# guo-research-group/Blurry-Edges

Hardware: AMD Instinct MI355X
Metric: patch-pairs/s (local CNN + render + depth) on 21x21 synth (higher is better)
Workload: dtype f32; 1 GPU; configs[1]: batch of 4096 synthetic 21x21 two-aperture patch pairs per GPU (8192 CNN patches): LocalStage inference + pass-A colour solve + depth solve; pairs_per_gpu=4096, streams=2, weights=portable-generator random init (no checkpoint offline)

## Files before the change

blurry-edges_amd/csrc/be_conv_pm_bf6.hip:

```cpp
#include "be_common.h"
#include "be_device_math.h"
#include "be_split_bf16.h"
#include <cstdlib>

namespace {

using be::bf6::bf16x8;
using be::bf6::f32x4;
using be::bf6::split8;
using be::bf6::PS_BLOCK;
using be::bf6::ps_slot;
typedef float f32x16 __attribute__((ext_vector_type(16)));
typedef __attribute__((address_space(3))) void* lds_ptr_t;
typedef const __attribute__((address_space(1))) void* glb_ptr_t;

constexpr int L0_BM = 128, L0_BKT = 16, L0_STAGES = 4;
constexpr int L0_ABYTES = L0_BM * L0_BKT * 4, L0_BBYTES = PS_BLOCK * 2, L0_STAGE = L0_ABYTES + L0_BBYTES;

struct PmBf6Args {
    const float* x;
    const float* x2;
    const float* planes;
    const float* bias;
    float* y;
    int Nimg, H, W, HW, Cin, Cin2, Cout, ldy, act, groups, ncc;
    int64_t istride, istride2;
};

__global__ __launch_bounds__(256, 2)
void k_conv_pm_bf6(PmBf6Args a) {
    constexpr int BM = L0_BM, BKT = L0_BKT, NS = L0_STAGES, ABYTES = L0_ABYTES, BBYTES = L0_BBYTES, STAGE = L0_STAGE;
    extern __shared__ __attribute__((aligned(16))) float smem_l0[];
    char* const lds = reinterpret_cast<char*>(smem_l0);

    const int bid = blockIdx.x;
    const int xcd = bid & 7, t = bid >> 3;
    const int grp = (t / a.HW) * 8 + xcd;
    if (grp >= a.groups) return;
    const int img0 = grp * BM;
    int py, px;
    {
        const int idx = t % a.HW, ni = (a.H - 2) * (a.W - 2);
        if (idx < ni) { py = 1 + idx / (a.W - 2); px = 1 + idx % (a.W - 2); }
        else {
            const int e = idx - ni;
            if (e < a.W) { py = 0; px = e; }
            else if (e < 2 * a.W) { py = a.H - 1; px = e - a.W; }
            else if (e < 2 * a.W + a.H - 2) { px = 0; py = 1 + e - 2 * a.W; }
            else { px = a.W - 1; py = 1 + e - 2 * a.W - (a.H - 2); }
        }
    }
    unsigned long long tap_list = 0;
    int ntap = 0;
#pragma unroll
    for (int k = 0; k < 9; ++k) {
        const bool ok = (unsigned)(py + k / 3 - 1) < (unsigned)a.H && (unsigned)(px + k % 3 - 1) < (unsigned)a.W;
        if (ok) { tap_list |= (unsigned long long)k << (4 * ntap); ++ntap; }
    }

    const int tid = threadIdx.x;
    const int wave = __builtin_amdgcn_readfirstlane(tid >> 6), lane = tid & 63;
    const int li = lane & 31, lh = lane >> 5;
    float bias_v[3];
#pragma unroll
    for (int j = 0; j < 3; ++j) {
        const int c = j * 32 + li;
        bias_v[j] = (c < a.Cout && a.bias) ? a.bias[c] : 0.0f;
    }
    const int srow = lane >> 2, sq = (lane & 3) ^ ((lane >> 4) & 3);
    unsigned a_off[2], a_off2[2];
#pragma unroll
    for (int p = 0; p < 2; ++p) {
        const int r = (2 * wave + p) * 16 + srow;
        const int rr = img0 + r < a.Nimg ? r : 0;
        a_off[p] = (unsigned)(rr * a.istride + 4 * sq) * 4u;
        a_off2[p] = (unsigned)(rr * a.istride2 + 4 * sq) * 4u;
    }
    const float* xpix = a.x + (int64_t)img0 * a.istride + (py * a.W + px) * a.Cin;
    const float* x2pix = a.x2 ? a.x2 + (int64_t)img0 * a.istride2 + (py * a.W + px) * a.Cin2 : nullptr;
    const char* wt = reinterpret_cast<const char*>(a.planes) + lane * 16;

    const int n_main = a.ncc * ntap * 2;
    const int total = n_main + (a.x2 ? a.Cin2 / BKT : 0);
    int w_cc = 0, w_j = 0, w_sub = 0, w_k = 0, l_buf = 0;
#define L0_DMA()                                                                                                \
    do {                                                                                                        \
        char* st_ = lds + l_buf * STAGE;                                                                        \
        const char* xs_;                                                                                        \
        int chunk_;                                                                                             \
        unsigned o0_, o1_;                                                                                      \
        if (w_k < n_main) {                                                                                     \
            const int tap_ = (int)((tap_list >> (4 * w_j)) & 15ull);                                            \
            const int ty_ = (tap_ * 11) >> 5, tx_ = tap_ - 3 * ty_;                         \
            xs_ = reinterpret_cast<const char*>(xpix + ((ty_ - 1) * a.W + tx_ - 1) * a.Cin + w_cc * 32 + w_sub * BKT); \
            chunk_ = (w_cc * 9 + tap_) * 2 + w_sub;                                                             \
            o0_ = a_off[0]; o1_ = a_off[1];                                                                     \
        } else {                                                                                                \
            const int k2_ = w_k - n_main;                                                                       \
            xs_ = reinterpret_cast<const char*>(x2pix + k2_ * BKT);                                             \
            chunk_ = a.ncc * 18 + k2_;                                                                          \
            o0_ = a_off2[0]; o1_ = a_off2[1];                                                                   \
        }                                                                                                       \
        __builtin_amdgcn_global_load_lds((glb_ptr_t)(xs_ + o0_), (lds_ptr_t)(st_ + (2 * wave) * 1024), 16, 0, 0);     \
        __builtin_amdgcn_global_load_lds((glb_ptr_t)(xs_ + o1_), (lds_ptr_t)(st_ + (2 * wave + 1) * 1024), 16, 0, 0); \
        const char* ws_ = wt + (int64_t)chunk_ * BBYTES;                                                        \
        _Pragma("unroll") for (int p_ = 0; p_ < 3; ++p_)                                                        \
            __builtin_amdgcn_global_load_lds((glb_ptr_t)(ws_ + (3 * wave + p_) * 1024),                         \
                                             (lds_ptr_t)(st_ + ABYTES + (3 * wave + p_) * 1024), 16, 0, 0);     \
        if (w_k + 1 < total) {                                           \
            ++w_k;                                                                                              \
            if (++w_sub == 2) { w_sub = 0; if (++w_j == ntap) { w_j = 0; ++w_cc; } }                            \
        }                                                                                                       \
        l_buf = (l_buf + 1) % NS;                                                                               \
    } while (0)

    const int fsw = (li >> 2) & 3;
    const int a_fr0 = ((wave * 32 + li) * BKT + 4 * ((2 * lh) ^ fsw)) * 4;
    const int a_fr1 = ((wave * 32 + li) * BKT + 4 * ((2 * lh + 1) ^ fsw)) * 4;
    const int b_fr = ABYTES + li * 32 + ps_slot(li, lh) * 16;
    f32x16 acc[3];
#pragma unroll
    for (int j = 0; j < 3; ++j)
#pragma unroll
        for (int r = 0; r < 16; ++r) acc[j][r] = 0.0f;
    bf16x8 ap[3], bp[3][3];
    int r_buf = 0;
#define L0_FRAGS()                                                                                              \
    do {                                                                                                        \
        const char* sb_ = lds + r_buf * STAGE;                                                                  \
        const f32x4 af0_ = *reinterpret_cast<const f32x4*>(sb_ + a_fr0);                                        \
        const f32x4 af1_ = *reinterpret_cast<const f32x4*>(sb_ + a_fr1);                                        \
        _Pragma("unroll") for (int p_ = 0; p_ < 3; ++p_)                                                        \
            _Pragma("unroll") for (int j_ = 0; j_ < 3; ++j_)                                                    \
                bp[p_][j_] = *reinterpret_cast<const bf16x8*>(sb_ + b_fr + p_ * 4096 + j_ * 32 * 32);           \
        split8(af0_, af1_, ap[0], ap[1], ap[2]);                                                                \
        r_buf = (r_buf + 1) % NS;                                                                               \
    } while (0)

    __builtin_amdgcn_sched_barrier(0);
    L0_DMA();
    L0_DMA();
    L0_DMA();
    __builtin_amdgcn_s_waitcnt(0x0F75);
    __builtin_amdgcn_s_barrier();
    L0_FRAGS();
    bool landed = true;
    for (int kc = 0; kc < total; ++kc) {
        if (!landed) __builtin_amdgcn_s_waitcnt(0x0F75);
        landed = false;
        __builtin_amdgcn_s_barrier();
        L0_DMA();
        __builtin_amdgcn_sched_barrier(0);
        {
            constexpr int PA[6] = {2, 0, 1, 1, 0, 0}, PB[6] = {0, 2, 1, 0, 1, 0};
#pragma unroll
            for (int p = 0; p < 6; ++p)
#pragma unroll
                for (int j = 0; j < 3; ++j)
                    acc[j] = __builtin_amdgcn_mfma_f32_32x32x16_bf16(ap[PA[p]], bp[PB[p]][j], acc[j], 0, 0, 0);
            L0_FRAGS();
        }
        __builtin_amdgcn_sched_barrier(0);
    }
#undef L0_DMA
#undef L0_FRAGS
    __builtin_amdgcn_s_waitcnt(0x0F70);
    __builtin_amdgcn_sched_barrier(0);

    const int64_t rs = (int64_t)a.HW * a.ldy;
    char* yt = reinterpret_cast<char*>(a.y + ((int64_t)img0 * a.HW + py * a.W + px) * a.ldy);
    const unsigned y_off = (unsigned)((wave * 32 + 4 * lh) * rs + li) * 4u;
    const bool interior = img0 + BM <= a.Nimg && a.Cout == 96;
#define L0_STORE(J)                                                                                             \
    do {                                                                                                        \
        float v_ = acc[J][r] + bias_v[J];                                                                       \
        if (a.act == 1) v_ = be::smish(v_); else if (a.act == 2) v_ = fmaxf(v_, 0.0f);                          \
        reinterpret_cast<float*>(yt + (size_t)ro * rs * 4 + y_off)[(J) * 32] = v_;                              \
    } while (0)
    if (interior) {
#pragma unroll
        for (int r = 0; r < 16; ++r) {
            const int ro = (r & 3) + 8 * (r >> 2);
#pragma unroll
            for (int j = 0; j < 3; ++j) L0_STORE(j);
        }
    } else {
#pragma unroll
        for (int j = 0; j < 3; ++j) {
            const bool c_ok = j * 32 + li < a.Cout;
#pragma unroll
            for (int r = 0; r < 16; ++r) {
                const int ro = (r & 3) + 8 * (r >> 2);
                if (c_ok && img0 + wave * 32 + 4 * lh + ro < a.Nimg) L0_STORE(j);
            }
        }
    }
#undef L0_STORE
}

inline int ktot_of(int cin, int cin2) { return 9 * cin + cin2; }
inline bool shape_ok(int cout, int cin, int cin2) {
    return cout > 0 && (cout + 31) / 32 * 32 == 96 && cin > 0 && cin % 32 == 0 && cin2 >= 0 && cin2 % 16 == 0;
}

}

bool be::l0_bf6_enabled() {
    static const bool f32 = (getenv("BE_L0_F32") != nullptr && atoi(getenv("BE_L0_F32")) != 0) ||
                            (getenv("BE_WINO_F32") != nullptr && atoi(getenv("BE_WINO_F32")) != 0);
    return !f32;
}

extern "C" size_t be_conv3x3_pm_bf6_packed_floats(int cout, int cin, int cin2) {
    if (!shape_ok(cout, cin, cin2)) return 0;
    return be_gemm_rows_bf6_packed_floats(cout, ktot_of(cin, cin2));
}

extern "C" int be_conv3x3_pm_bf6_pack_f32(const float* packed_w, int cout, int cin, int cin2, float* planes, void* stream) {
    BE_REQUIRE(packed_w && planes, "be_conv3x3_pm_bf6_pack_f32: null pointer");
    BE_REQUIRE(shape_ok(cout, cin, cin2),
               "be_conv3x3_pm_bf6_pack_f32: unsupported shape (cout %d: cout_pad32 must be 96; cin %d %% 32; cin2 %d %% 16)", cout, cin, cin2);
    return be_gemm_rows_bf6_pack_f32(packed_w, cout, ktot_of(cin, cin2), planes, stream);
}

int be::conv3x3_pm_bf6(const be_conv_desc* d, const float* x, const float* x2, int cin2, const float* planes, const float* bias,
                       float* y, int ldy, void* stream) {
    BE_REQUIRE(d && x && planes && y, "be_conv3x3_pm_bf6_f32: null pointer");
    BE_REQUIRE(d->ksize == 3 && d->n >= 0 && (unsigned)d->act <= 2u, "be_conv3x3_pm_bf6_f32: bad descriptor (ksize %d, n %d, act %d)",
               d->ksize, d->n, d->act);
    BE_REQUIRE(x2 || cin2 == 0, "be_conv3x3_pm_bf6_f32: cin2 %d without x2", cin2);
    BE_REQUIRE(shape_ok(d->cout, d->cin, cin2) && (!x2 || cin2 > 0),
               "be_conv3x3_pm_bf6_f32: unsupported shape (cout %d: cout_pad32 must be 96; cin %d %% 32; cin2 %d %% 16)", d->cout, d->cin, cin2);
    BE_REQUIRE(d->h >= 3 && d->w >= 3 && ldy >= d->cout, "be_conv3x3_pm_bf6_f32: unsupported map (h %d, w %d >= 3; ldy %d >= cout)",
               d->h, d->w, ldy);
    BE_REQUIRE(be::aligned16(x) && be::aligned16(x2) && be::aligned16(planes) && (reinterpret_cast<uintptr_t>(y) & 3u) == 0 &&
               (!bias || (reinterpret_cast<uintptr_t>(bias) & 3u) == 0),
               "be_conv3x3_pm_bf6_f32: x / x2 / planes must be 16-byte aligned, y / bias 4-byte");
    if (d->n == 0) return BE_OK;
    PmBf6Args a;
    a.x = x; a.x2 = x2; a.planes = planes; a.bias = bias; a.y = y;
    a.Nimg = d->n; a.H = d->h; a.W = d->w; a.HW = d->h * d->w; a.Cin = d->cin; a.Cin2 = x2 ? cin2 : 0; a.Cout = d->cout; a.ldy = ldy;
    a.act = d->act; a.ncc = d->cin / 32;
    a.istride = (int64_t)a.HW * d->cin;
    a.istride2 = (int64_t)a.HW * a.Cin2;
    const int64_t span = 256 * 4 * (a.istride > a.istride2 ? a.istride : a.istride2);
    BE_REQUIRE(span < ((int64_t)1 << 32) && 256 * 4 * (int64_t)a.HW * ldy < ((int64_t)1 << 32),
               "be_conv3x3_pm_bf6_f32: 256 images must span < 2^32 bytes");
    a.groups = (d->n + L0_BM - 1) / L0_BM;
// ... 29 lines not shown
```

blurry-edges_amd/csrc/be_split_bf16.h:

```cpp
#pragma once
#include <hip/hip_runtime.h>

namespace be {
namespace bf6 {

typedef float f32x4 __attribute__((ext_vector_type(4)));
typedef float f32x2 __attribute__((ext_vector_type(2)));
typedef __bf16 bf16x8 __attribute__((ext_vector_type(8)));
typedef __bf16 bf16x2 __attribute__((ext_vector_type(2)));

__device__ __forceinline__ float bf_lo(unsigned u) { return __uint_as_float(u << 16); }
__device__ __forceinline__ float bf_hi(unsigned u) { return __uint_as_float(u & 0xffff0000u); }
__device__ __forceinline__ float sub_f32(float x, float y) {
    float r;
    asm("v_sub_f32 %0, %1, %2" : "=v"(r) : "v"(x), "v"(y));
    return r;
}
__device__ __forceinline__ void split8(f32x4 a, f32x4 b, bf16x8& h, bf16x8& m, bf16x8& l) {
    const float x[8] = {a.x, a.y, a.z, a.w, b.x, b.y, b.z, b.w};
#pragma unroll
    for (int e = 0; e < 8; e += 2) {
        const bf16x2 hb = __builtin_convertvector((f32x2){x[e], x[e + 1]}, bf16x2);
        const unsigned hu = __builtin_bit_cast(unsigned, hb);
        const float r0 = sub_f32(x[e], bf_lo(hu)), r1 = sub_f32(x[e + 1], bf_hi(hu));
        const bf16x2 mb = __builtin_convertvector((f32x2){r0, r1}, bf16x2);
        const unsigned mu = __builtin_bit_cast(unsigned, mb);
        const bf16x2 lb = __builtin_convertvector((f32x2){sub_f32(r0, bf_lo(mu)), sub_f32(r1, bf_hi(mu))}, bf16x2);
        h[e] = hb[0]; h[e + 1] = hb[1];
        m[e] = mb[0]; m[e + 1] = mb[1];
        l[e] = lb[0]; l[e + 1] = lb[1];
    }
}

typedef __bf16 bf16x4 __attribute__((ext_vector_type(4)));
__device__ __forceinline__ void split4(f32x4 a, bf16x4& h, bf16x4& m, bf16x4& l) {
    const float x[4] = {a.x, a.y, a.z, a.w};
#pragma unroll
    for (int e = 0; e < 4; e += 2) {
        const bf16x2 hb = __builtin_convertvector((f32x2){x[e], x[e + 1]}, bf16x2);
        const unsigned hu = __builtin_bit_cast(unsigned, hb);
        const float r0 = sub_f32(x[e], bf_lo(hu)), r1 = sub_f32(x[e + 1], bf_hi(hu));
        const bf16x2 mb = __builtin_convertvector((f32x2){r0, r1}, bf16x2);
        const unsigned mu = __builtin_bit_cast(unsigned, mb);
        const bf16x2 lb = __builtin_convertvector((f32x2){sub_f32(r0, bf_lo(mu)), sub_f32(r1, bf_hi(mu))}, bf16x2);
        h[e] = hb[0]; h[e + 1] = hb[1];
        m[e] = mb[0]; m[e + 1] = mb[1];
        l[e] = lb[0]; l[e + 1] = lb[1];
    }
}

constexpr int PS_BLOCK = 3 * 128 * 16;
__device__ __forceinline__ int ps_slot(int row, int half) { return half ^ ((row >> 3) & 1); }

}
}
```

blurry-edges_amd/csrc/be_wino.hip:

```cpp
#include <algorithm>
#include <cstdint>
#include <cstdlib>
#include "be_common.h"
#include "be_device_math.h"
#include "be_split_bf16.h"
#include "be_wino_math.h"

namespace {

typedef float f32x4 __attribute__((ext_vector_type(4)));

constexpr int TH = be::WINO_TH, NR = be::WINO_NR, TY = be::WINO_TY, TPI = be::WINO_TPI, NPOS = be::WINO_NPOS, NOUT = be::WINO_OUT;

inline unsigned grid_cap(int64_t total, int block, int64_t limit = 65535) {
    int64_t g = (total + block - 1) / block;
    return (unsigned)(g < 1 ? 1 : (g > limit ? limit : g));
}

__global__ void k_wino_pack(const float* __restrict__ w, const float* __restrict__ b, const float* __restrict__ gamma,
                            const float* __restrict__ beta, const float* __restrict__ mean, const float* __restrict__ var,
                            float eps, int cout, int cin, int cout_pad, float* __restrict__ U, float* __restrict__ bias) {
    const int64_t total = (int64_t)cout_pad * cin;
    const int64_t gs = (int64_t)gridDim.x * blockDim.x;
    for (int64_t idx = (int64_t)blockIdx.x * blockDim.x + threadIdx.x; idx < total; idx += gs) {
// ... 164 lines not shown
                    for (int c = 0; c < 5; ++c) {
                        const int yy = TH * ty - 1 + r, xx = 3 * tx - 1 + c;
                        d[r][c] = (xx >= 0 && xx < 6 && yy >= 0 && yy < 6) ? y[yy < 0 ? 0 : (yy > 5 ? 5 : yy)][xx < 0 ? 0 : (xx > 5 ? 5 : xx)] : zero;
                    }
                be::wino_in(d, v);
                vec* dst = reinterpret_cast<vec*>(V) + (img * TPI + ty * 2 + tx) * ts_o + cq;
#pragma unroll
                for (int z = 0; z < NPOS; ++z) st_s<NT>(dst + (size_t)z * plane_o, v[z]);
            }
    }
}

template <int NT, int VW = VW_OUT>
__global__ __launch_bounds__(256, VW_OUT == 2 ? 2 : 1)
void k_wino_out_pool2(const float* __restrict__ M, const float* __restrict__ bias, const float* __restrict__ res,
                      float* __restrict__ y, int64_t n, int c4, int act, int tm) {
    typedef typename VecOf<VW>::type vec;
    const int64_t total = n * c4;
    const int64_t gs = (int64_t)gridDim.x * blockDim.x;
    const int64_t plane = tm ? c4 : n * TPI * c4, ts = tm ? NPOS * c4 : c4;
    for (int64_t idx = (int64_t)blockIdx.x * blockDim.x + threadIdx.x; idx < total; idx += gs) {
        const int cq = (int)(idx % c4);
        const int64_t img = idx / c4;
        const vec bv = reinterpret_cast<const vec*>(bias)[cq];
        vec v[6][6];
#pragma unroll
        for (int ty = 0; ty < TY; ++ty)
#pragma unroll
            for (int tx = 0; tx < 2; ++tx) {
                const vec* src = reinterpret_cast<const vec*>(M) + (img * TPI + ty * 2 + tx) * ts + cq;
                vec m[NPOS], o[NOUT], rv[NOUT];
#pragma unroll
                for (int z = 0; z < NPOS; ++z) m[z] = ld_s<NT>(src + (size_t)z * plane);
                if (res) {
#pragma unroll
                    for (int r = 0; r < TH; ++r)
#pragma unroll
                        for (int c = 0; c < 3; ++c)
                            rv[3 * r + c] = ld_s<NT>(reinterpret_cast<const vec*>(res) + ((size_t)img * 36 + (TH * ty + r) * 6 + 3 * tx + c) * c4 + cq);
                }
                be::wino_out(m, o);
#pragma unroll
                for (int r = 0; r < TH; ++r)
#pragma unroll
                    for (int c = 0; c < 3; ++c) {
                        vec w = o[3 * r + c] + bv;
                        if (res) w += rv[3 * r + c];
                        v[TH * ty + r][3 * tx + c] = wino_act(w, act);
                    }
            }
#pragma unroll
        for (int py = 0; py < 3; ++py)
#pragma unroll
            for (int px = 0; px < 3; ++px) {
                vec m;
#pragma unroll
                for (int k = 0; k < VW; ++k)
                    m[k] = fmaxf(fmaxf(v[2 * py][2 * px][k], v[2 * py][2 * px + 1][k]), fmaxf(v[2 * py + 1][2 * px][k], v[2 * py + 1][2 * px + 1][k]));
                st_s<NT>(reinterpret_cast<vec*>(y) + ((size_t)img * 9 + py * 3 + px) * c4 + cq, m);
            }
    }
}

typedef float f32x16 __attribute__((ext_vector_type(16)));
typedef __attribute__((address_space(3))) void* lds_ptr_t;
typedef const __attribute__((address_space(1))) void* glb_ptr_t;

struct GemmArgs {
    const float* x;
    const float* w;
    float* y;
    int M, K, N, ldy, nb, m_tiles, n_tiles;
    int64_t xb, wb, yb;
    int lda;
    int mrows, zrows;
    const float* bias;
    const float* res;
    int act;
    int zgroups;
    int npad;
};

using be::bf6::bf16x8;
using be::bf6::split8;
using be::bf6::PS_BLOCK;
using be::bf6::ps_slot;

constexpr int PS_STAGES = 4;

__global__ void k_wino_pack_split(const float* __restrict__ U, int npos, int cout_pad, int cin, int n_tiles, __bf16* __restrict__ P) {
    const int kg = cin / 8, rows = 128 * n_tiles;
    const int64_t total = (int64_t)npos * rows * kg;
    const int64_t gs = (int64_t)gridDim.x * blockDim.x;
    for (int64_t idx = (int64_t)blockIdx.x * blockDim.x + threadIdx.x; idx < total; idx += gs) {
        const int g = (int)(idx % kg), row = (int)((idx / kg) % rows), z = (int)(idx / ((int64_t)kg * rows));
        f32x4 lo4 = {0.f, 0.f, 0.f, 0.f}, hi4 = lo4;
        if (row < cout_pad) {
            const f32x4* src = reinterpret_cast<const f32x4*>(U + ((size_t)z * cout_pad + row) * cin + 8 * g);
            lo4 = src[0];
            hi4 = src[1];
        }
        bf16x8 h, m, l;
        split8(lo4, hi4, h, m, l);
        const int r = row & 127;
        bf16x8* dst = reinterpret_cast<bf16x8*>(P + ((size_t)(z * n_tiles + (row >> 7)) * (cin / 16) + (g >> 1)) * PS_BLOCK) + 2 * r +
                      ps_slot(r, g & 1);
        dst[0] = h;
        dst[256] = m;
        dst[512] = l;
    }
}

template <int EPI, int BF6 = 0>
__global__ __launch_bounds__(256, 3)
void k_wino_gemm(GemmArgs a) {
    constexpr int BM = 128, BN = 128, BKT = 16;
    constexpr int STAGE = (BM + BN) * BKT;
    extern __shared__ __attribute__((aligned(16))) float smem_w[];
    const int bid = blockIdx.x;
    const int xcd = bid & 7, slot = bid >> 3;
    const int n_tile = slot % a.n_tiles;
    int m_tile = (slot / a.n_tiles) * 8 + xcd;
    if constexpr (BF6) {
        const int zg = m_tile % a.zgroups, zper = (a.nb + a.zgroups - 1) / a.zgroups;
        m_tile /= a.zgroups;
        if (m_tile >= a.m_tiles || zg * zper >= a.nb) return;
        a.x += (int64_t)zg * zper * a.xb;
        a.w += (int64_t)zg * zper * a.wb;
        a.y += (int64_t)zg * zper * a.yb;
        a.nb = min(zper, a.nb - zg * zper);
    }
    if (m_tile >= a.m_tiles) return;
    const int n0 = n_tile * BN, row_base = m_tile * a.mrows;
    const int tid = threadIdx.x;
    const int wave = __builtin_amdgcn_readfirstlane(tid >> 6), lane = tid & 63;
    const int wm = wave >> 1, wn = wave & 1;
    const int li = lane & 31, lh = lane >> 5;
    const int srow = lane >> 2, sq = (lane & 3) ^ ((lane >> 4) & 3);
    unsigned a_off[2], b_off[2];
#pragma unroll
    for (int p = 0; p < 2; ++p) {
        const int r = (2 * wave + p) * 16 + srow;
        a_off[p] = (unsigned)((row_base + r < a.M ? r : 0) * a.lda + 4 * sq) * 4u;
        b_off[p] = (unsigned)(r * a.K + 4 * sq) * 4u;
        if (BF6 && n0 + r >= a.npad) b_off[p] = (unsigned)(4 * sq) * 4u;
    }
    const float* xt = a.x + (int64_t)row_base * a.lda;
    const float* wt = a.w + (int64_t)n0 * a.K;
    const int kchunks = a.K / BKT, total = kchunks * a.nb;
    const int fsw = (li >> 2) & 3;
    const int q0 = BF6 ? 2 * lh : lh, q1 = BF6 ? 2 * lh + 1 : lh + 2;
    const int a_fr0 = (wm * 64 + li) * BKT + 4 * (q0 ^ fsw);
    const int a_fr1 = (wm * 64 + li) * BKT + 4 * (q1 ^ fsw);
    const int b_fr0 = BM * BKT + (wn * 64 + li) * BKT + 4 * (q0 ^ fsw);
    const int b_fr1 = BM * BKT + (wn * 64 + li) * BKT + 4 * (q1 ^ fsw);
    f32x16 acc[2][2];
#pragma unroll
    for (int i = 0; i < 2; ++i)
#pragma unroll
        for (int j = 0; j < 2; ++j)
#pragma unroll
            for (int r = 0; r < 16; ++r) acc[i][j][r] = 0.0f;
    int lz = 0, lk = 0;
#define WG_LOAD(BUF)                                                                                            \
    do {                                                                                                        \
        const char* xs_ = reinterpret_cast<const char*>(xt + (int64_t)lz * a.xb + lk * BKT);                     \
// ... 102 lines not shown
                                reinterpret_cast<float*>(yt + (size_t)ro * a.ldy * 4 + y_off)[j * 32] = v_;
                            }
                        }
                }
            }
#undef WG_VALUE
#pragma unroll
            for (int i = 0; i < 2; ++i)
#pragma unroll
                for (int j = 0; j < 2; ++j)
#pragma unroll
                    for (int r = 0; r < 16; ++r) acc[i][j][r] = 0.0f;
            ck = 0; ++cz;
        }
    }
#undef WG_LOAD
}

template <int EPI, int ROWS = 0>
__global__ __launch_bounds__(256, 2)
void k_wino_gemm_ps(GemmArgs a) {
    constexpr int BM = 128, BKT = 16;
    constexpr int ABYTES = BM * BKT * 4, BBYTES = PS_BLOCK * 2, STAGE = ABYTES + BBYTES;
    constexpr int NS = PS_STAGES;
    extern __shared__ __attribute__((aligned(16))) float smem_w[];
    char* const lds = reinterpret_cast<char*>(smem_w);
    const int bid = blockIdx.x;
    const int xcd = bid & 7, slot = bid >> 3;
    const int n_tile = slot % a.n_tiles;
    int m_tile = (slot / a.n_tiles) * 8 + xcd;
    const int zg = m_tile % a.zgroups, zper = (a.nb + a.zgroups - 1) / a.zgroups;
    m_tile /= a.zgroups;
    if (m_tile >= a.m_tiles || zg * zper >= a.nb) return;
    const int nb = min(zper, a.nb - zg * zper), kchunks = a.K / BKT, total = kchunks * nb;
    const int n0 = n_tile * 128, row_base = m_tile * (ROWS ? a.mrows : BM);
    const int tid = threadIdx.x;
    const int wave = __builtin_amdgcn_readfirstlane(tid >> 6), lane = tid & 63;
    const int wm = wave >> 1, wn = wave & 1;
    const int li = lane & 31, lh = lane >> 5;
    const int srow = lane >> 2, sq = (lane & 3) ^ ((lane >> 4) & 3);
    unsigned a_off[2];
#pragma unroll
    for (int p = 0; p < 2; ++p) {
        const int r = (2 * wave + p) * 16 + srow;
        a_off[p] = (unsigned)((row_base + r < a.M ? r : 0) * a.lda + 4 * sq) * 4u;
    }
    const char* xt = reinterpret_cast<const char*>(a.x + (int64_t)zg * zper * a.xb + (int64_t)row_base * a.lda);
    const char* wt = reinterpret_cast<const char*>(a.w + (int64_t)zg * zper * a.wb) + (int64_t)n_tile * kchunks * BBYTES + lane * 16;
    float* const yg = a.y + (int64_t)zg * zper * a.yb;
    const int fsw = (li >> 2) & 3;
    const int a_fr0 = ((wm * 64 + li) * BKT + 4 * ((2 * lh) ^ fsw)) * 4;
    const int a_fr1 = ((wm * 64 + li) * BKT + 4 * ((2 * lh + 1) ^ fsw)) * 4;
    const int b_fr = ABYTES + (wn * 64 + li) * 32 + ps_slot(li, lh) * 16;
    f32x16 acc[2][2];
#pragma unroll
    for (int i = 0; i < 2; ++i)
#pragma unroll
        for (int j = 0; j < 2; ++j)
#pragma unroll
            for (int r = 0; r < 16; ++r) acc[i][j][r] = 0.0f;
    int lz = 0, lk = 0, l_buf = 0;
#define PS_DMA()                                                                                                \
    do {                                                                                                        \
        const char* xs_ = xt + ((int64_t)lz * a.xb + lk * BKT) * 4;                                             \
        const char* ws_ = wt + (int64_t)lz * a.wb * 4 + lk * BBYTES;                                            \
        char* st_ = lds + l_buf * STAGE;                                                                        \
        _Pragma("unroll") for (int p_ = 0; p_ < 2; ++p_)                                                        \
            __builtin_amdgcn_global_load_lds((glb_ptr_t)(xs_ + a_off[p_]), (lds_ptr_t)(st_ + (2 * wave + p_) * 1024), 16, 0, 0); \
        _Pragma("unroll") for (int p_ = 0; p_ < 3; ++p_)                                                        \
            __builtin_amdgcn_global_load_lds((glb_ptr_t)(ws_ + (3 * wave + p_) * 1024),                         \
                                             (lds_ptr_t)(st_ + ABYTES + (3 * wave + p_) * 1024), 16, 0, 0);     \
        if (lk + 1 < kchunks) ++lk; else if (lz + 1 < nb) { lk = 0; ++lz; }    \
        l_buf = (l_buf + 1) % NS;                                                                               \
    } while (0)
    const unsigned y_off = (unsigned)((wm * 64 + 4 * lh) * a.ldy + wn * 64 + li) * 4u;
    float bias_v[2] = {0.f, 0.f};
    if (EPI) {
#pragma unroll
        for (int j = 0; j < 2; ++j) {
            const int c = n0 + wn * 64 + j * 32 + li;
            bias_v[j] = (a.bias && c < a.N) ? a.bias[c] : 0.0f;
        }
    }
    bf16x8 ap[3][2], bp[3][2];
    int r_buf = 0;
#define PS_FRAGS()                                                                                              \
    do {                                                                                                        \
        const char* sb_ = lds + r_buf * STAGE;                                                                  \
        f32x4 af_[2][2];                                                                                        \
        _Pragma("unroll") for (int i_ = 0; i_ < 2; ++i_) {                                                      \
            af_[0][i_] = *reinterpret_cast<const f32x4*>(sb_ + a_fr0 + i_ * 32 * BKT * 4);                      \
            af_[1][i_] = *reinterpret_cast<const f32x4*>(sb_ + a_fr1 + i_ * 32 * BKT * 4);                      \
        }                                                                                                       \
        _Pragma("unroll") for (int p_ = 0; p_ < 3; ++p_)                                                        \
            _Pragma("unroll") for (int j_ = 0; j_ < 2; ++j_)                                                    \
                bp[p_][j_] = *reinterpret_cast<const bf16x8*>(sb_ + b_fr + p_ * 4096 + j_ * 32 * 32);           \
        _Pragma("unroll") for (int i_ = 0; i_ < 2; ++i_) split8(af_[0][i_], af_[1][i_], ap[0][i_], ap[1][i_], ap[2][i_]); \
        r_buf = (r_buf + 1) % NS;                                                                               \
    } while (0)
    PS_DMA();
    PS_DMA();
    PS_DMA();
    __builtin_amdgcn_s_waitcnt(0x0F75);
    __builtin_amdgcn_s_barrier();
    PS_FRAGS();
    int cz = 0, ck = 0;
    bool landed = true;
    for (int kc = 0; kc < total; ++kc) {
        if (!landed) __builtin_amdgcn_s_waitcnt(0x0F75);
        landed = false;
        __builtin_amdgcn_s_barrier();
        PS_DMA();
        __builtin_amdgcn_sched_barrier(0);
        {
            constexpr int PA[6] = {2, 0, 1, 1, 0, 0}, PB[6] = {0, 2, 1, 0, 1, 0};
#pragma unroll
            for (int p = 0; p < 6; ++p)
#pragma unroll
                for (int i = 0; i < 2; ++i)
#pragma unroll
                    for (int j = 0; j < 2; ++j)
                        acc[i][j] = __builtin_amdgcn_mfma_f32_32x32x16_bf16(ap[PA[p]][i], bp[PB[p]][j], acc[i][j], 0, 0, 0);
            PS_FRAGS();
        }
        __builtin_amdgcn_sched_barrier(0);
        if (++ck == kchunks) {
            if (kc + 1 < total) __builtin_amdgcn_s_waitcnt(0x0F75);
            else __builtin_amdgcn_s_waitcnt(0x0F70);
            landed = true;
            __builtin_amdgcn_sched_barrier(0);
            const int zrow = ROWS ? row_base + cz * a.zrows : row_base;
            char* yt = reinterpret_cast<char*>(yg + (int64_t)cz * a.yb + (int64_t)row_base * a.ldy + n0);
            const char* rt = EPI && a.res ? reinterpret_cast<const char*>(a.res) + (yt - reinterpret_cast<char*>(a.y)) : nullptr;
#define PS_VALUE(J)                                                                                             \
            float v_ = acc[i][J][r];                                                                            \
            if (EPI) {                                                                                          \
                v_ += bias_v[J];                                                                                \
                if (rt) v_ += reinterpret_cast<const float*>(rt + (size_t)ro * a.ldy * 4 + y_off)[(J) * 32];    \
                if (a.act == 1) v_ = be::smish(v_); else if (a.act == 2) v_ = fmaxf(v_, 0.0f);                  \
            }
            if (zrow + BM <= a.M && n0 + 128 <= a.N) {
#pragma unroll
                for (int i = 0; i < 2; ++i)
#pragma unroll
                    for (int r = 0; r < 16; ++r) {
                        const int ro = i * 32 + (r & 3) + 8 * (r >> 2);
                        float* yr = reinterpret_cast<float*>(yt + (size_t)ro * a.ldy * 4 + y_off);
                        { PS_VALUE(0) yr[0] = v_; }
                        { PS_VALUE(1) yr[32] = v_; }
                    }
            } else {
#pragma unroll
                for (int j = 0; j < 2; ++j) {
                    const bool c_ok = n0 + wn * 64 + j * 32 + li < a.N;
#pragma unroll
                    for (int i = 0; i < 2; ++i)
#pragma unroll
                        for (int r = 0; r < 16; ++r) {
                            const int ro = i * 32 + (r & 3) + 8 * (r >> 2);
                            if (c_ok && zrow + wm * 64 + 4 * lh + ro < a.M) {
                                PS_VALUE(j)
                                reinterpret_cast<float*>(yt + (size_t)ro * a.ldy * 4 + y_off)[j * 32] = v_;
                            }
                        }
                }
            }
#undef PS_VALUE
#pragma unroll
            for (int i = 0; i < 2; ++i)
#pragma unroll
                for (int j = 0; j < 2; ++j)
#pragma unroll
                    for (int r = 0; r < 16; ++r) acc[i][j][r] = 0.0f;
            ck = 0; ++cz;
        }
    }
#undef PS_DMA
#undef PS_FRAGS
}

template <int KCH, int KIND>
__global__ __launch_bounds__(256, 1)
void k_wino_gemm_ws(GemmArgs a, int mgroups) {
    constexpr int BM = 128, BKT = 16, ABUF = BM * BKT;
    extern __shared__ __attribute__((aligned(16))) float smem_w[];
    const int bid = blockIdx.x;
    const int xcd = bid & 7, slot = bid >> 3;
    const int n_tile = slot % a.n_tiles;
    const int unit = (slot / a.n_tiles) * 8 + xcd;
    const int z = unit / mgroups, mg = unit % mgroups;
    const int tiles_per = (a.m_tiles + mgroups - 1) / mgroups;
    const int t0 = mg * tiles_per, t1 = min(a.m_tiles, t0 + tiles_per);
    if (z >= a.nb || t0 >= t1) return;
    const int n0 = n_tile * 128;
    const int tid = threadIdx.x;
    const int wave = __builtin_amdgcn_readfirstlane(tid >> 6), lane = tid & 63;
    const int wm = wave >> 1, wn = wave & 1;
    const int li = lane & 31, lh = lane >> 5;
    const int srow = lane >> 2, sq = (lane & 3) ^ ((lane >> 4) & 3);
    const int fsw = (li >> 2) & 3;
    const int fr0 = li * BKT + 4 * (lh ^ fsw), fr1 = li * BKT + 4 * ((lh + 2) ^ fsw);
    f32x4 breg[KCH][2][2];
    {
        constexpr int PASS = 8;
        const float* wt = a.w + (int64_t)z * a.wb + (int64_t)n0 * a.K;
        unsigned b_off[2];
#pragma unroll
        for (int p = 0; p < 2; ++p) b_off[p] = (unsigned)(((2 * wave + p) * 16 + srow) * a.K + 4 * sq) * 4u;
#pragma unroll
        for (int c0 = 0; c0 < KCH; c0 += PASS) {
#pragma unroll
            for (int cc = 0; cc < PASS; ++cc)
                if (c0 + cc < KCH) {
#pragma unroll
                    for (int p = 0; p < 2; ++p)
                        __builtin_amdgcn_global_load_lds((glb_ptr_t)(reinterpret_cast<const char*>(wt + (c0 + cc) * BKT) + b_off[p]),
                                                         (lds_ptr_t)(smem_w + cc * ABUF + (2 * wave + p) * 256), 16, 0, 0);
                }
            __syncthreads();
#pragma unroll
            for (int cc = 0; cc < PASS; ++cc)
                if (c0 + cc < KCH) {
                    const float* st = smem_w + cc * ABUF;
#pragma unroll
                    for (int j = 0; j < 2; ++j) {
                        breg[c0 + cc][0][j] = *reinterpret_cast<const f32x4*>(st + (wn * 64 + j * 32) * BKT + fr0);
                        breg[c0 + cc][1][j] = *reinterpret_cast<const f32x4*>(st + (wn * 64 + j * 32) * BKT + fr1);
                    }
                }
            __syncthreads();
        }
    }
    unsigned a_off[2];
#pragma unroll
    for (int p = 0; p < 2; ++p) a_off[p] = (unsigned)(((2 * wave + p) * 16 + srow) * a.lda + 4 * sq) * 4u;
    const float* xz = a.x + (int64_t)z * a.xb;
    int l_tile = t0, l_c = 0, l_buf = 0;
#define WS_DMA()                                                                                                \
    do {                                                                                                        \
        const int lt_ = l_tile < t1 ? l_tile : t1 - 1;                         \
        const char* xs_ = reinterpret_cast<const char*>(xz + (int64_t)lt_ * BM * a.lda + l_c * BKT);            \
        float* st_ = smem_w + l_buf * ABUF + (2 * wave) * 256;                                                  \
        _Pragma("unroll") for (int p_ = 0; p_ < 2; ++p_)                                                        \
            __builtin_amdgcn_global_load_lds((glb_ptr_t)(xs_ + a_off[p_]), (lds_ptr_t)(st_ + p_ * 256), 16, 0, 0); \
        if (++l_c == KCH) { l_c = 0; ++l_tile; }                                                                \
        l_buf = l_buf == 2 ? 0 : l_buf + 1;                                                                     \
    } while (0)
    f32x16 acc[2][2];
#pragma unroll
    for (int i = 0; i < 2; ++i)
#pragma unroll
        for (int j = 0; j < 2; ++j)
#pragma unroll
            for (int r = 0; r < 16; ++r) acc[i][j][r] = 0.0f;
    f32x4 fa[2][2][2];
    WS_DMA();
    WS_DMA();
    __builtin_amdgcn_s_waitcnt(0x0F72);
    __builtin_amdgcn_s_barrier();
    int r_buf = 0;
#define WS_READ(SET)                                                                                            \
// ... 429 lines not shown
```

Baseline: 429,200 patch-pairs/s.

## Interleave LDS fragment loads and bf16 splitting with MFMA issue via register double-buffering

The conv and Winograd GEMM main loops now double-buffer the A/B fragment registers and unroll by two. The LDS reads and the three-way bf16 split for the next k-chunk are spread between individual MFMA instructions using sched_barrier, so they no longer sit serially after the MFMA burst. The split helpers are restructured into per-pair functions that pack directly into u32 lanes. This raises register pressure, and the EPI path of the Winograd kernel keeps the old serial schedule.

```diff
diff --git a/blurry-edges_amd/csrc/be_conv_pm_bf6.hip b/blurry-edges_amd/csrc/be_conv_pm_bf6.hip
--- a/blurry-edges_amd/csrc/be_conv_pm_bf6.hip
+++ b/blurry-edges_amd/csrc/be_conv_pm_bf6.hip
@@ -8,6 +8,7 @@
 using be::bf6::bf16x8;
 using be::bf6::f32x4;
 using be::bf6::split8;
+using be::bf6::u32x4;
 using be::bf6::PS_BLOCK;
 using be::bf6::ps_slot;
 typedef float f32x16 __attribute__((ext_vector_type(16)));
@@ -123,17 +124,41 @@
     for (int j = 0; j < 3; ++j)
 #pragma unroll
         for (int r = 0; r < 16; ++r) acc[j][r] = 0.0f;
-    bf16x8 ap[3], bp[3][3];
+    u32x4 ap[2][3];
+    bf16x8 bp[2][3][3];
     int r_buf = 0;
-#define L0_FRAGS()                                                                                              \
+#define L0_CHUNK(S)                                                                                             \
     do {                                                                                                        \
+        constexpr int PA[6] = {2, 0, 1, 1, 0, 0}, PB[6] = {0, 2, 1, 0, 1, 0};                                   \
         const char* sb_ = lds + r_buf * STAGE;                                                                  \
-        const f32x4 af0_ = *reinterpret_cast<const f32x4*>(sb_ + a_fr0);                                        \
-        const f32x4 af1_ = *reinterpret_cast<const f32x4*>(sb_ + a_fr1);                                        \
-        _Pragma("unroll") for (int p_ = 0; p_ < 3; ++p_)                                                        \
-            _Pragma("unroll") for (int j_ = 0; j_ < 3; ++j_)                                                    \
-                bp[p_][j_] = *reinterpret_cast<const bf16x8*>(sb_ + b_fr + p_ * 4096 + j_ * 32 * 32);           \
-        split8(af0_, af1_, ap[0], ap[1], ap[2]);                                                                \
+        f32x4 af_[2];                                                                               \
+        float r0_[4], r1_[4];                                                                                   \
+        _Pragma("unroll") for (int g_ = 0; g_ < 18; ++g_) {                                                     \
+            acc[g_ % 3] = __builtin_amdgcn_mfma_f32_32x32x16_bf16(__builtin_bit_cast(bf16x8, ap[S][PA[g_ / 3]]),\
+                                                                  bp[S][PB[g_ / 3]][g_ % 3], acc[g_ % 3], 0, 0, 0); \
+            if (g_ == 0) {                                                                                      \
+                af_[0] = *reinterpret_cast<const f32x4*>(sb_ + a_fr0);                                          \
+                af_[1] = *reinterpret_cast<const f32x4*>(sb_ + a_fr1);                                          \
+            }                                                                                                   \
+            if (g_ >= 1 && g_ < 6)                                                                              \
+                _Pragma("unroll") for (int b_ = 2 * (g_ - 1); b_ < 2 * g_ && b_ < 9; ++b_)                      \
+                    bp[(S) ^ 1][b_ / 3][b_ % 3] =                                                               \
+                        *reinterpret_cast<const bf16x8*>(sb_ + b_fr + (b_ / 3) * 4096 + (b_ % 3) * 32 * 32);    \
+            if (g_ >= 10) {                                                                                     \
+                const int u_ = (g_ - 10) >> 1;                                                                  \
+                if ((g_ & 1) == 0) {                                                                            \
+                    unsigned h_, m_;                                                                            \
+                    be::bf6::split_pair_a(af_[u_ >> 1][(2 * u_) & 3], af_[u_ >> 1][(2 * u_ + 1) & 3], h_, m_, r0_[u_], r1_[u_]); \
+                    ap[(S) ^ 1][0][u_] = h_;                                                                    \
+                    ap[(S) ^ 1][1][u_] = m_;                                                                    \
+                } else {                                                                                        \
+                    unsigned l_ = be::bf6::split_pair_b(r0_[u_], r1_[u_], ap[(S) ^ 1][1][u_]);                  \
+                    asm volatile("" : "+v"(l_));                      \
+                    ap[(S) ^ 1][2][u_] = l_;                                                                    \
+                }                                                                                               \
+            }                                                                                                   \
+            __builtin_amdgcn_sched_barrier(0);                                                                  \
+        }                                                                                                       \
         r_buf = (r_buf + 1) % NS;                                                                               \
     } while (0)
 
@@ -143,27 +168,42 @@
     L0_DMA();
     __builtin_amdgcn_s_waitcnt(0x0F75);
     __builtin_amdgcn_s_barrier();
-    L0_FRAGS();
+    {
+        const f32x4 af0_ = *reinterpret_cast<const f32x4*>(lds + a_fr0);
+        const f32x4 af1_ = *reinterpret_cast<const f32x4*>(lds + a_fr1);
+#pragma unroll
+        for (int p = 0; p < 3; ++p)
+#pragma unroll
+            for (int j = 0; j < 3; ++j) bp[0][p][j] = *reinterpret_cast<const bf16x8*>(lds + b_fr + p * 4096 + j * 32 * 32);
+        bf16x8 h, m, l;
+        split8(af0_, af1_, h, m, l);
+        ap[0][0] = __builtin_bit_cast(u32x4, h);
+        ap[0][1] = __builtin_bit_cast(u32x4, m);
+        ap[0][2] = __builtin_bit_cast(u32x4, l);
+        r_buf = 1;
+    }
     bool landed = true;
-    for (int kc = 0; kc < total; ++kc) {
-        if (!landed) __builtin_amdgcn_s_waitcnt(0x0F75);
-        landed = false;
-        __builtin_amdgcn_s_barrier();
-        L0_DMA();
+#define L0_TOP()                                                                                                \
+    do {                                                                                                        \
+        if (!landed) __builtin_amdgcn_s_waitcnt(0x0F75);                                \
+        landed = false;                                                                                         \
+        __builtin_amdgcn_s_barrier();                   \
+        L0_DMA();                                                                \
+        __builtin_amdgcn_sched_barrier(0);                                                                      \
+    } while (0)
+    for (int kc = 0; kc < total; kc += 2) {
+        L0_TOP();
+        L0_CHUNK(0);
         __builtin_amdgcn_sched_barrier(0);
-        {
-            constexpr int PA[6] = {2, 0, 1, 1, 0, 0}, PB[6] = {0, 2, 1, 0, 1, 0};
-#pragma unroll
-            for (int p = 0; p < 6; ++p)
-#pragma unroll
-                for (int j = 0; j < 3; ++j)
-                    acc[j] = __builtin_amdgcn_mfma_f32_32x32x16_bf16(ap[PA[p]], bp[PB[p]][j], acc[j], 0, 0, 0);
-            L0_FRAGS();
+        if (kc + 1 < total) {
+            L0_TOP();
+            L0_CHUNK(1);
+            __builtin_amdgcn_sched_barrier(0);
         }
-        __builtin_amdgcn_sched_barrier(0);
-    }
+    }
+#undef L0_TOP
 #undef L0_DMA
-#undef L0_FRAGS
+#undef L0_CHUNK
     __builtin_amdgcn_s_waitcnt(0x0F70);
     __builtin_amdgcn_sched_barrier(0);
 
diff --git a/blurry-edges_amd/csrc/be_split_bf16.h b/blurry-edges_amd/csrc/be_split_bf16.h
--- a/blurry-edges_amd/csrc/be_split_bf16.h
+++ b/blurry-edges_amd/csrc/be_split_bf16.h
@@ -16,37 +16,49 @@
     asm("v_sub_f32 %0, %1, %2" : "=v"(r) : "v"(x), "v"(y));
     return r;
 }
+typedef unsigned u32x4 __attribute__((ext_vector_type(4)));
+typedef unsigned u32x2 __attribute__((ext_vector_type(2)));
+__device__ __forceinline__ void split_pair_a(float x0, float x1, unsigned& hu, unsigned& mu, float& r0, float& r1) {
+    hu = __builtin_bit_cast(unsigned, __builtin_convertvector((f32x2){x0, x1}, bf16x2));
+    r0 = sub_f32(x0, bf_lo(hu));
+    r1 = sub_f32(x1, bf_hi(hu));
+    mu = __builtin_bit_cast(unsigned, __builtin_convertvector((f32x2){r0, r1}, bf16x2));
+}
+__device__ __forceinline__ unsigned split_pair_b(float r0, float r1, unsigned mu) {
+    return __builtin_bit_cast(unsigned, __builtin_convertvector((f32x2){sub_f32(r0, bf_lo(mu)), sub_f32(r1, bf_hi(mu))}, bf16x2));
+}
+
 __device__ __forceinline__ void split8(f32x4 a, f32x4 b, bf16x8& h, bf16x8& m, bf16x8& l) {
     const float x[8] = {a.x, a.y, a.z, a.w, b.x, b.y, b.z, b.w};
+    u32x4 hu, mu, lu;
 #pragma unroll
-    for (int e = 0; e < 8; e += 2) {
-        const bf16x2 hb = __builtin_convertvector((f32x2){x[e], x[e + 1]}, bf16x2);
-        const unsigned hu = __builtin_bit_cast(unsigned, hb);
-        const float r0 = sub_f32(x[e], bf_lo(hu)), r1 = sub_f32(x[e + 1], bf_hi(hu));
-        const bf16x2 mb = __builtin_convertvector((f32x2){r0, r1}, bf16x2);
-        const unsigned mu = __builtin_bit_cast(unsigned, mb);
-        const bf16x2 lb = __builtin_convertvector((f32x2){sub_f32(r0, bf_lo(mu)), sub_f32(r1, bf_hi(mu))}, bf16x2);
-        h[e] = hb[0]; h[e + 1] = hb[1];
-        m[e] = mb[0]; m[e + 1] = mb[1];
-        l[e] = lb[0]; l[e + 1] = lb[1];
+    for (int u = 0; u < 4; ++u) {
+        float r0, r1;
+        unsigned h_, m_;
+        split_pair_a(x[2 * u], x[2 * u + 1], h_, m_, r0, r1);
+        hu[u] = h_; mu[u] = m_;
+        lu[u] = split_pair_b(r0, r1, m_);
     }
+    h = __builtin_bit_cast(bf16x8, hu);
+    m = __builtin_bit_cast(bf16x8, mu);
+    l = __builtin_bit_cast(bf16x8, lu);
 }
 
 typedef __bf16 bf16x4 __attribute__((ext_vector_type(4)));
 __device__ __forceinline__ void split4(f32x4 a, bf16x4& h, bf16x4& m, bf16x4& l) {
     const float x[4] = {a.x, a.y, a.z, a.w};
+    u32x2 hu, mu, lu;
 #pragma unroll
-    for (int e = 0; e < 4; e += 2) {
-        const bf16x2 hb = __builtin_convertvector((f32x2){x[e], x[e + 1]}, bf16x2);
-        const unsigned hu = __builtin_bit_cast(unsigned, hb);
-        const float r0 = sub_f32(x[e], bf_lo(hu)), r1 = sub_f32(x[e + 1], bf_hi(hu));
-        const bf16x2 mb = __builtin_convertvector((f32x2){r0, r1}, bf16x2);
-        const unsigned mu = __builtin_bit_cast(unsigned, mb);
-        const bf16x2 lb = __builtin_convertvector((f32x2){sub_f32(r0, bf_lo(mu)), sub_f32(r1, bf_hi(mu))}, bf16x2);
-        h[e] = hb[0]; h[e + 1] = hb[1];
-        m[e] = mb[0]; m[e + 1] = mb[1];
-        l[e] = lb[0]; l[e + 1] = lb[1];
+    for (int u = 0; u < 2; ++u) {
+        float r0, r1;
+        unsigned h_, m_;
+        split_pair_a(x[2 * u], x[2 * u + 1], h_, m_, r0, r1);
+        hu[u] = h_; mu[u] = m_;
+        lu[u] = split_pair_b(r0, r1, m_);
     }
+    h = __builtin_bit_cast(bf16x4, hu);
+    m = __builtin_bit_cast(bf16x4, mu);
+    l = __builtin_bit_cast(bf16x4, lu);
 }
 
 constexpr int PS_BLOCK = 3 * 128 * 16;
diff --git a/blurry-edges_amd/csrc/be_wino.hip b/blurry-edges_amd/csrc/be_wino.hip
--- a/blurry-edges_amd/csrc/be_wino.hip
+++ b/blurry-edges_amd/csrc/be_wino.hip
@@ -270,6 +270,7 @@
 };
 
 using be::bf6::bf16x8;
+using be::bf6::u32x4;
 using be::bf6::split8;
 using be::bf6::PS_BLOCK;
 using be::bf6::ps_slot;
@@ -538,11 +539,46 @@
             bias_v[j] = (a.bias && c < a.N) ? a.bias[c] : 0.0f;
         }
     }
-    bf16x8 ap[3][2], bp[3][2];
+    u32x4 ap[2][3][2];
+    bf16x8 bp[2][3][2];
     int r_buf = 0;
-#define PS_FRAGS()                                                                                              \
+#define PS_CHUNK(S)                                                                                             \
     do {                                                                                                        \
+        constexpr int PA[6] = {2, 0, 1, 1, 0, 0}, PB[6] = {0, 2, 1, 0, 1, 0};                                   \
         const char* sb_ = lds + r_buf * STAGE;                                                                  \
+        f32x4 af_[2][2];                                                                         \
+        float r0_[8], r1_[8];                                                                                   \
+        _Pragma("unroll") for (int g_ = 0; g_ < 24; ++g_) {                                                     \
+            acc[(g_ >> 1) & 1][g_ & 1] = __builtin_amdgcn_mfma_f32_32x32x16_bf16(                               \
+                __builtin_bit_cast(bf16x8, ap[S][PA[g_ >> 2]][(g_ >> 1) & 1]), bp[S][PB[g_ >> 2]][g_ & 1],      \
+                acc[(g_ >> 1) & 1][g_ & 1], 0, 0, 0);                                                           \
+            if (g_ < 2) {                                                                                       \
+                af_[0][g_] = *reinterpret_cast<const f32x4*>(sb_ + a_fr0 + g_ * 32 * BKT * 4);                  \
+                af_[1][g_] = *reinterpret_cast<const f32x4*>(sb_ + a_fr1 + g_ * 32 * BKT * 4);                  \
+            }                                                                                                   \
+            if (g_ >= 2 && g_ < 5)                                                                              \
+                _Pragma("unroll") for (int j_ = 0; j_ < 2; ++j_)                                                \
+                    bp[(S) ^ 1][g_ - 2][j_] = *reinterpret_cast<const bf16x8*>(sb_ + b_fr + (g_ - 2) * 4096 + j_ * 32 * 32); \
+            if (g_ >= 8) {                                                                                      \
+                const int u_ = (g_ - 8) >> 1, i_ = u_ >> 2, e_ = u_ & 3;                                        \
+                if ((g_ & 1) == 0) {                                                                            \
+                    unsigned h_, m_;                                                                            \
+                    be::bf6::split_pair_a(af_[e_ >> 1][i_][(2 * e_) & 3], af_[e_ >> 1][i_][(2 * e_ + 1) & 3], h_, m_, r0_[u_], r1_[u_]); \
+                    ap[(S) ^ 1][0][i_][e_] = h_;                                                                \
+                    ap[(S) ^ 1][1][i_][e_] = m_;                                                                \
+                } else {                                                                                        \
+                    unsigned l_ = be::bf6::split_pair_b(r0_[u_], r1_[u_], ap[(S) ^ 1][1][i_][e_]);              \
+                    asm volatile("" : "+v"(l_));                      \
+                    ap[(S) ^ 1][2][i_][e_] = l_;                                                                \
+                }                                                                                               \
+            }                                                                                                   \
+            __builtin_amdgcn_sched_barrier(0);                                                                  \
+        }                                                                                                       \
+        r_buf = (r_buf + 1) % NS;                                                                               \
+    } while (0)
+#define PS_FRAGS0(SLOT)                                                                                         \
+    do {                                                                                                        \
+        const char* sb_ = lds + (SLOT) * STAGE;                                                                 \
         f32x4 af_[2][2];                                                                                        \
         _Pragma("unroll") for (int i_ = 0; i_ < 2; ++i_) {                                                      \
             af_[0][i_] = *reinterpret_cast<const f32x4*>(sb_ + a_fr0 + i_ * 32 * BKT * 4);                      \
@@ -550,36 +586,33 @@
         }                                                                                                       \
         _Pragma("unroll") for (int p_ = 0; p_ < 3; ++p_)                                                        \
             _Pragma("unroll") for (int j_ = 0; j_ < 2; ++j_)                                                    \
-                bp[p_][j_] = *reinterpret_cast<const bf16x8*>(sb_ + b_fr + p_ * 4096 + j_ * 32 * 32);           \
-        _Pragma("unroll") for (int i_ = 0; i_ < 2; ++i_) split8(af_[0][i_], af_[1][i_], ap[0][i_], ap[1][i_], ap[2][i_]); \
-        r_buf = (r_buf + 1) % NS;                                                                               \
+                bp[0][p_][j_] = *reinterpret_cast<const bf16x8*>(sb_ + b_fr + p_ * 4096 + j_ * 32 * 32);        \
+        _Pragma("unroll") for (int i_ = 0; i_ < 2; ++i_) {                                                      \
+            bf16x8 h_, m_, l_;                                                                                  \
+            split8(af_[0][i_], af_[1][i_], h_, m_, l_);                                                         \
+            ap[0][0][i_] = __builtin_bit_cast(u32x4, h_);                                                       \
+            ap[0][1][i_] = __builtin_bit_cast(u32x4, m_);                                                       \
+            ap[0][2][i_] = __builtin_bit_cast(u32x4, l_);                                                       \
+        }                                                                                                       \
     } while (0)
     PS_DMA();
     PS_DMA();
     PS_DMA();
     __builtin_amdgcn_s_waitcnt(0x0F75);
     __builtin_amdgcn_s_barrier();
-    PS_FRAGS();
+    PS_FRAGS0(0);
+    r_buf = 1;
     int cz = 0, ck = 0;
     bool landed = true;
-    for (int kc = 0; kc < total; ++kc) {
-        if (!landed) __builtin_amdgcn_s_waitcnt(0x0F75);
-        landed = false;
-        __builtin_amdgcn_s_barrier();
-        PS_DMA();
-        __builtin_amdgcn_sched_barrier(0);
-        {
-            constexpr int PA[6] = {2, 0, 1, 1, 0, 0}, PB[6] = {0, 2, 1, 0, 1, 0};
-#pragma unroll
-            for (int p = 0; p < 6; ++p)
-#pragma unroll
-                for (int i = 0; i < 2; ++i)
-#pragma unroll
-                    for (int j = 0; j < 2; ++j)
-                        acc[i][j] = __builtin_amdgcn_mfma_f32_32x32x16_bf16(ap[PA[p]][i], bp[PB[p]][j], acc[i][j], 0, 0, 0);
-            PS_FRAGS();
-        }
-        __builtin_amdgcn_sched_barrier(0);
+#define PS_TOP()                                                                                                \
+    do {                                                                                                        \
+        if (!landed) __builtin_amdgcn_s_waitcnt(0x0F75);                                \
+        landed = false;                                                                                         \
+        __builtin_amdgcn_s_barrier();                   \
+        PS_DMA();                                                                \
+        __builtin_amdgcn_sched_barrier(0);                                                                      \
+    } while (0)
+    auto boundary = [&](int kc) __attribute__((always_inline)) {
         if (++ck == kchunks) {
             if (kc + 1 < total) __builtin_amdgcn_s_waitcnt(0x0F75);
             else __builtin_amdgcn_s_waitcnt(0x0F70);
@@ -630,9 +663,44 @@
                     for (int r = 0; r < 16; ++r) acc[i][j][r] = 0.0f;
             ck = 0; ++cz;
         }
-    }
+    };
+    if constexpr (EPI) {
+        for (int kc = 0; kc < total; ++kc) {
+            PS_TOP();
+            {
+                constexpr int PA[6] = {2, 0, 1, 1, 0, 0}, PB[6] = {0, 2, 1, 0, 1, 0};
+#pragma unroll
+                for (int p = 0; p < 6; ++p)
+#pragma unroll
+                    for (int i = 0; i < 2; ++i)
+#pragma unroll
+                        for (int j = 0; j < 2; ++j)
+                            acc[i][j] = __builtin_amdgcn_mfma_f32_32x32x16_bf16(__builtin_bit_cast(bf16x8, ap[0][PA[p]][i]), bp[0][PB[p]][j],
+                                                                                acc[i][j], 0, 0, 0);
+                PS_FRAGS0(r_buf);
+                r_buf = (r_buf + 1) % NS;
+            }
+            __builtin_amdgcn_sched_barrier(0);
+            boundary(kc);
+        }
+    } else {
+        for (int kc = 0; kc < total; kc += 2) {
+            PS_TOP();
+            PS_CHUNK(0);
+            __builtin_amdgcn_sched_barrier(0);
+            boundary(kc);
+            if (kc + 1 < total) {
+                PS_TOP();
+                PS_CHUNK(1);
+                __builtin_amdgcn_sched_barrier(0);
+                boundary(kc + 1);
+            }
+        }
+    }
+#undef PS_TOP
 #undef PS_DMA
-#undef PS_FRAGS
+#undef PS_FRAGS0
+#undef PS_CHUNK
 }
 
 template <int KCH, int KIND>
```

Measured after the change: 435,800 patch-pairs/s (median of 6 runs). 1.5% higher.
